# facebookresearch/pytorch3d

Measured on NVIDIA H100. Metric: rasterize frames/sec (fwd+bwd) 512^2 K=8, higher is better.
Workload: dtype f32

## Files before the change

### pytorch3d_b200/csrc/raster_meshes.cu

```cuda
#include <cfloat>
#include <climits>

#include "binning.cuh"
#include "bulk_copy.cuh"
#include "common.cuh"
#include "raster_math.cuh"

namespace b200r {

constexpr int SETUP_FACES = 256;
#ifndef B200R_MESH_TILE_H
#define B200R_MESH_TILE_H 16
#endif
constexpr int FTW = 16, FTH = B200R_MESH_TILE_H, FTHREADS = FTW * FTH;
static_assert(FTH == 16 || FTH == 8, "16x16 or 16x8 tiles");
constexpr int CHUNK = FTHREADS;
constexpr int SMEMQ_MAX_K = 32;

__device__ __forceinline__ bool face_is_drawable(const Face& f, bool cull_backfaces) {
  const float zmax = fmaxf(fmaxf(f.z0, f.z1), f.z2), zmin = fminf(fminf(f.z0, f.z1), f.z2);
  if (!(zmax >= 0.0f)) return false;
  if ((double)zmin < kEps) return false;
  const float area = edge_fn(f.x0, f.y0, f.x1, f.y1, f.x2, f.y2);
  if (cull_backfaces && area < 0.0f) return false;
// ... 916 lines not shown
      }
      store_pair_run<3 * KMAX / 4>(reinterpret_cast<float4*>(p.bary + oa * 3), piece, odd, vA, vB);
    }
    stored = true;
   }
  }
  if (!stored && valid) {
#pragma unroll
    for (int k = 0; k < KMAX; ++k) {
      if (k < K) {
        const bool e = k >= q.size;
        const float4 w = e ? make_float4(-1.f, -1.f, -1.f, -1.f) : pay[slot[k] * FTHREADS];
        p.pix_to_face[o + k] = e ? -1ll : (long long)q.id[k];
        p.zbuf[o + k] = e ? -1.0f : q.z[k];
        p.dists[o + k] = w.x;
        p.bary[(o + k) * 3 + 0] = w.y;
        p.bary[(o + k) * 3 + 1] = w.z;
        p.bary[(o + k) * 3 + 2] = w.w;
      }
    }
  }
  if (order != ORDER_ARRIVAL || !tile_saw_tie(sh)) return;
  order = ORDER_INDEX;
  rq.reset();
  }
}

__device__ __forceinline__ void recompute_hit(const FineParams& p, int fi, float px, float py, Hit& h) {
  const float4* r = p.rec + (int64_t)fi * 4;
  const float4 fa = __ldg(r + 0), fb = __ldg(r + 1), fc = __ldg(r + 2);
  const Face f = {fa.x, fa.y, fc.x, fa.z, fa.w, fc.y, fb.x, fb.y, fc.z};
  eval_pixel_face<false>(px, py, f, fb.z, p.blur_radius, p.persp != 0, p.clip != 0, false, 0.0f, h);
}

template <bool NB, bool SCAN>
__global__ void __launch_bounds__(FTHREADS, SCAN ? B200R_SMEMQ_SCAN_CTAS : B200R_SMEMQ_CTAS) mesh_fine_smemq_kernel(const FineParams p) {
  extern __shared__ __align__(16) unsigned char smem_raw[];
  FineStage& sh = *reinterpret_cast<FineStage*>(smem_raw);
  const int tid = threadIdx.x, lane = tid & 31;
  const TileWork t = tile_work(p);
  const int tile_x = t.tile_x, tile_y = t.tile_y, n = t.n;
  if (t.count == 0) {
    write_empty_tile<0>(p, n, tile_x, tile_y);
    return;
  }
  int xo, yo;
  fthread_pixel(tile_x, tile_y, xo, yo);
  const bool valid = xo < p.W && yo < p.H;
  const int lc = xo - tile_x * FTW, lr = yo - tile_y * FTH;
  const int K = p.K;

  SmemQueue<NB> q;
  q.init(smem_raw + sizeof(FineStage), K, tid);
  int order = first_walk_order<NB, SCAN>(p, t);
  bool active = valid;
  int scratch_ints = p.smem_ints;
  for (;;) {
  fine_tile_body<SmemQueue<NB>, NB, SCAN>(p, sh, q, tile_x, tile_y, n, t.seg_begin, t.count, t.overflow, order, active,
                                          scratch_ints, lc, lr);
  if (order == ORDER_DEPTH) {
    if (tile_saw_tie(sh)) {
      active = valid && sh.tie_lane[tid] != 0;
      if (active) q.reset();
      order = ORDER_INDEX;
      scratch_ints = (int)(sizeof(FineStage) / sizeof(int));
      __syncthreads();
      continue;
    }
  }
  q.sort();
  const float px = sh.col[lc], py = sh.row[lr];
  const int64_t o = (((int64_t)n * p.H + yo) * p.W + xo) * K;
  if ((K & 7) == 0) {
    const int odd = lane & 1;
    const bool vA = __shfl_sync(0xffffffffu, (int)valid, lane & ~1) != 0;
    const bool vB = __shfl_sync(0xffffffffu, (int)valid, lane | 1) != 0;
    const int64_t oa = o - (int64_t)odd * K, ob = oa + K;
    for (int g = 0; g < K; g += 8) {
      float4 pi[4], pzv[2], pd[2], pb[6];
      float z[8], d[8], b[24];
      int id[8];
#pragma unroll
      for (int u = 0; u < 8; ++u) {
        Hit h = {-1.0f, -1.0f, -1.0f, -1.0f, -1.0f};
        id[u] = -1;
        if (g + u < q.size) {
          id[u] = q.qi[(g + u) * FTHREADS];
          recompute_hit(p, id[u], px, py, h);
        }
        z[u] = h.z;
        d[u] = h.dist;
        b[3 * u + 0] = h.b0;
        b[3 * u + 1] = h.b1;
        b[3 * u + 2] = h.b2;
      }
#pragma unroll
      for (int u = 0; u < 4; ++u)
        pi[u] = make_float4(__int_as_float(id[2 * u]), __int_as_float(id[2 * u] >> 31),
                            __int_as_float(id[2 * u + 1]), __int_as_float(id[2 * u + 1] >> 31));
#pragma unroll
      for (int u = 0; u < 2; ++u) {
        pzv[u] = make_float4(z[4 * u], z[4 * u + 1], z[4 * u + 2], z[4 * u + 3]);
        pd[u] = make_float4(d[4 * u], d[4 * u + 1], d[4 * u + 2], d[4 * u + 3]);
      }
#pragma unroll
      for (int u = 0; u < 6; ++u) pb[u] = make_float4(b[4 * u], b[4 * u + 1], b[4 * u + 2], b[4 * u + 3]);
      store_pair_split<4>(reinterpret_cast<float4*>(p.pix_to_face + oa + g),
                          reinterpret_cast<float4*>(p.pix_to_face + ob + g), pi, odd, vA, vB);
      store_pair_split<2>(reinterpret_cast<float4*>(p.zbuf + oa + g), reinterpret_cast<float4*>(p.zbuf + ob + g), pzv,
                          odd, vA, vB);
      store_pair_split<2>(reinterpret_cast<float4*>(p.dists + oa + g), reinterpret_cast<float4*>(p.dists + ob + g),
                          pd, odd, vA, vB);
      store_pair_split<6>(reinterpret_cast<float4*>(p.bary + (oa + g) * 3),
                          reinterpret_cast<float4*>(p.bary + (ob + g) * 3), pb, odd, vA, vB);
    }
  } else if (valid) {
  for (int k = 0; k < K; ++k) {
    Hit h = {-1.0f, -1.0f, -1.0f, -1.0f, -1.0f};
    long long id = -1;
    if (k < q.size) {
      const int fi = q.qi[k * FTHREADS];
      recompute_hit(p, fi, px, py, h);
      id = fi;
    }
    p.pix_to_face[o + k] = id;
    p.zbuf[o + k] = h.z;
    p.dists[o + k] = h.dist;
    p.bary[(o + k) * 3 + 0] = h.b0;
    p.bary[(o + k) * 3 + 1] = h.b1;
    p.bary[(o + k) * 3 + 2] = h.b2;
  }
  }
  if (order != ORDER_ARRIVAL || !tile_saw_tie(sh)) return;
  order = ORDER_INDEX;
  q.reset();
  }
}

__global__ void __launch_bounds__(FTHREADS) mesh_fine_bigk_kernel(const FineParams p) {
  __shared__ FaceChunk s;
  const int tid = threadIdx.x, lane = tid & 31;
  const int t = blockIdx.x;
  const int n = t / (p.TY * p.TX);
  const int tile_y = (t / p.TX) % p.TY, tile_x = t % p.TX;
  int xo, yo;
  fthread_pixel(tile_x, tile_y, xo, yo);
  const bool valid = xo < p.W && yo < p.H;
  const float px = pix_to_ndc(p.W - 1 - xo, p.W, p.rx);
  const float py = pix_to_ndc(p.H - 1 - yo, p.H, p.ry);
  const float fx_lo = warp_min(valid ? px : FLT_MAX), fx_hi = warp_max(valid ? px : -FLT_MAX);
  const float fy_lo = warp_min(valid ? py : FLT_MAX), fy_hi = warp_max(valid ? py : -FLT_MAX);
  pdl_wait();
  const int seg_begin = p.tile_offset[t], seg_end = p.tile_offset[t + 1];
  const bool overflow = (int64_t)seg_end > p.capacity || seg_end == INT_MAX;
  const int64_t mesh_first = p.first[n];
  const int count = overflow ? (int)p.num[n] : seg_end - seg_begin;
  const bool persp = p.persp != 0, clip = p.clip != 0, cull = p.cull != 0;
  const int K = p.K;

  if (!overflow && count > 1)
    cta_sort_segment<FTHREADS>(p.pairs + seg_begin, count, reinterpret_cast<int*>(&s),
                               (int)(sizeof(FaceChunk) / sizeof(int)));

  float qz[B200R_MAX_K], qd[B200R_MAX_K];
  int qi[B200R_MAX_K];
  int qn = 0, q_max_idx = -1;
  float q_max_z = -1000.0f;

  for (int base = 0; base < count; base += CHUNK) {
    const int nc = min(CHUNK, count - base);
    __syncthreads();
    if (tid < nc) {
      const int f = overflow ? (int)(mesh_first + base + tid) : p.pairs[seg_begin + base + tid];
      stage_face(s, tid, p.face_verts, p.neighbor, f, p.sqrt_blur, cull);
    }
    __syncthreads();
    for (int g = 0; g < nc; g += 32) {
      bool touch = false;
      if (g + lane < nc) {
        const float4 bx = s.box[g + lane];
        touch = !(fx_lo > bx.y || fx_hi < bx.x || fy_lo > bx.w || fy_hi < bx.z);
      }
      unsigned m = __ballot_sync(0xffffffffu, touch);
      while (m) {
        const int j = g + __ffs(m) - 1;
        m &= m - 1;
        const float4 bx = s.box[j];
        if (!valid || px > bx.y || px < bx.x || py > bx.w || py < bx.z) continue;
        const float4 fa = s.a[j], fb = s.b[j], fc = s.c[j];
        const Face f = {fa.x, fa.y, fc.x, fa.z, fa.w, fc.y, fb.x, fb.y, fc.z};
        Hit h;
        const int nb = __float_as_int(fc.w);
        if (!eval_pixel_face<false>(px, py, f, fb.z, p.blur_radius, persp, clip, qn >= K && nb == -1, q_max_z, h))
          continue;
        const int fi = __float_as_int(fb.w);
        int at = -1;
        if (nb != -1)
          for (int i = 0; i < qn; ++i)
            if (qi[i] == nb) {
              at = i;
              break;
            }
        if (at >= 0) {
          if (fabsf(h.dist) < fabsf(qd[at])) {
            qz[at] = h.z;
            qi[at] = fi;
            qd[at] = h.dist;
            if (h.z > q_max_z) {
              q_max_z = h.z;
              q_max_idx = at;
            }
          }
        } else if (qn < K) {
          qz[qn] = h.z;
          qi[qn] = fi;
          qd[qn] = h.dist;
          if (h.z > q_max_z) {
            q_max_z = h.z;
            q_max_idx = qn;
          }
          ++qn;
        } else if (h.z < q_max_z) {
          qz[q_max_idx] = h.z;
          qi[q_max_idx] = fi;
          qd[q_max_idx] = h.dist;
          q_max_z = h.z;
          for (int i = 0; i < K; ++i)
            if (qz[i] > q_max_z) {
              q_max_z = qz[i];
              q_max_idx = i;
            }
        }
      }
    }
  }
  if (!valid) return;
  for (int i = 1; i < qn; ++i) {
    const float tz = qz[i];
    const int ti = qi[i];
    int j = i - 1;
    while (j >= 0 && key_less(tz, ti, qz[j], qi[j])) {
      qz[j + 1] = qz[j];
      qi[j + 1] = qi[j];
      --j;
    }
    qz[j + 1] = tz;
    qi[j + 1] = ti;
  }
  const int64_t o = (((int64_t)n * p.H + yo) * p.W + xo) * K;
  for (int k = 0; k < K; ++k) {
    Hit h = {-1.0f, -1.0f, -1.0f, -1.0f, -1.0f};
    long long id = -1;
    if (k < qn) {
      const float* v = p.face_verts + (int64_t)qi[k] * 9;
      const Face f = {__ldg(v + 0), __ldg(v + 1), __ldg(v + 2), __ldg(v + 3), __ldg(v + 4),
                      __ldg(v + 5), __ldg(v + 6), __ldg(v + 7), __ldg(v + 8)};
      eval_pixel_face<false>(px, py, f, bary_denominator(f), p.blur_radius, persp, clip, false, 0.0f, h);
      id = qi[k];
    }
    p.pix_to_face[o + k] = id;
    p.zbuf[o + k] = h.z;
    p.dists[o + k] = h.dist;
    p.bary[(o + k) * 3 + 0] = h.b0;
    p.bary[(o + k) * 3 + 1] = h.b1;
    p.bary[(o + k) * 3 + 2] = h.b2;
  }
}

struct BackwardParams {
  const float* face_verts;
  const int64_t* pix_to_face;
  const float* grad_zbuf;
  const float* grad_bary;
  const float* grad_dists;
  int N, H, W, K, TY, TX;
  int n0;
  int g_vec;
  int64_t F;
  float rx, ry;
  int persp, clip;
  float* grad_face_verts;
  const int64_t* faces;
  float* grad_verts;
  int64_t V;
};

__device__ __forceinline__ void edge_bwd(float px, float py, float ax, float ay, float bx, float by, float g,
                                         float2& dp, float2& da, float2& db) {
  dp = make_float2(g * (by - ay), g * (ax - bx));
  da = make_float2(g * (py - by), g * (bx - px));
  db = make_float2(g * (ay - py), g * (px - ax));
}

__device__ __forceinline__ void point_line_bwd(float px, float py, float ax, float ay, float bx, float by, float g,
                                               float2& ga, float2& gb) {
  const float bax = bx - ax, bay = by - ay;
  const float t = __saturatef((bax * (px - ax) + bay * (py - ay)) / (bax * bax + bay * bay));
  const float qx = (1.0f - t) * ax + t * bx, qy = (1.0f - t) * ay + t * by;
  const float cx = 2.0f * (qx - px), cy = 2.0f * (qy - py);
  ga = make_float2(g * (1.0f - t) * cx, g * (1.0f - t) * cy);
  gb = make_float2(g * t * cx, g * t * cy);
}

__device__ __forceinline__ void backward_one(const BackwardParams& p, float px, float py, int64_t fi, float gz,
                                             float gd, float gb0, float gb1, float gb2, bool persp, bool clip,
                                             float (&out)[9]) {
  const float* v = p.face_verts + fi * 9;
  const Face f = {__ldg(v + 0), __ldg(v + 1), __ldg(v + 2), __ldg(v + 3), __ldg(v + 4),
                  __ldg(v + 5), __ldg(v + 6), __ldg(v + 7), __ldg(v + 8)};
  const float den = bary_denominator(f);
  float w0, w1, w2;
  bary_coords(px, py, f, den, w0, w1, w2);
  float c0 = w0, c1 = w1, c2 = w2;
  if (persp) bary_persp(c0, c1, c2, f.z0, f.z1, f.z2);
  float k0 = c0, k1 = c1, k2 = c2;
  if (clip) bary_clip(k0, k1, k2);
  const bool inside = c0 > 0.0f && c1 > 0.0f && c2 > 0.0f;
  const float sgd = inside ? -gd : gd;

  float2 dv0 = make_float2(0.f, 0.f), dv1 = dv0, dv2 = dv0;
  {
    const float e01 = point_line_dist(px, py, f.x0, f.y0, f.x1, f.y1);
    const float e02 = point_line_dist(px, py, f.x0, f.y0, f.x2, f.y2);
    const float e12 = point_line_dist(px, py, f.x1, f.y1, f.x2, f.y2);
    if (e01 <= e02 && e01 <= e12)
      point_line_bwd(px, py, f.x0, f.y0, f.x1, f.y1, sgd, dv0, dv1);
    else if (e02 <= e01 && e02 <= e12)
      point_line_bwd(px, py, f.x0, f.y0, f.x2, f.y2, sgd, dv0, dv2);
    else if (e12 <= e01 && e12 <= e02)
      point_line_bwd(px, py, f.x1, f.y1, f.x2, f.y2, sgd, dv1, dv2);
  }

  float g0 = gb0 + gz * f.z0, g1 = gb1 + gz * f.z1, g2 = gb2 + gz * f.z2;
  if (clip) {
    const float m0 = fmaxf(c0, 0.0f), m1 = fmaxf(c1, 0.0f), m2 = fmaxf(c2, 0.0f);
    float sum = m0 + m1 + m2, gsc = 1.0f;
    if (sum < 1e-5f) {
      gsc = 0.0f;
      sum = 1e-5f;
    }
    const float inv = __frcp_rn(sum), inv2 = gsc * inv * inv;
    const float s0 = -m0 * inv2, s1 = -m1 * inv2, s2 = -m2 * inv2;
    const float cross = g0 * s0 + g1 * s1 + g2 * s2;
    const float n0 = c0 < 0.0f ? 0.0f : g0 * inv + cross;
    const float n1 = c1 < 0.0f ? 0.0f : g1 * inv + cross;
    const float n2 = c2 < 0.0f ? 0.0f : g2 * inv + cross;
    g0 = n0;
    g1 = n1;
    g2 = n2;
  }
  float dz0 = 0.0f, dz1 = 0.0f, dz2 = 0.0f;
  if (persp) {
    const float t0 = w0 * f.z1 * f.z2, t1 = f.z0 * w1 * f.z2, t2 = f.z0 * f.z1 * w2;
    const float dn = fmaxf(t0 + t1 + t2, 1e-8f);
    const float rdn = __frcp_rn(dn);
    const float gdn = (-t0 * g0 - t1 * g1 - t2 * g2) * rdn * rdn;
    const float h0 = gdn + g0 * rdn, h1 = gdn + g1 * rdn, h2 = gdn + g2 * rdn;
    g0 = h0 * f.z1 * f.z2;
    g1 = h1 * f.z0 * f.z2;
    g2 = h2 * f.z0 * f.z1;
    dz0 = h1 * w1 * f.z2 + h2 * w2 * f.z1;
    dz1 = h0 * w0 * f.z2 + h2 * w2 * f.z0;
    dz2 = h0 * w0 * f.z1 + h1 * w1 * f.z0;
  }
  float2 bv0 = make_float2(0.f, 0.f), bv1 = bv0, bv2 = bv0;
  {
    const float rden = __frcp_rn(den);
    const float e0 = edge_fn(px, py, f.x1, f.y1, f.x2, f.y2);
    const float e1 = edge_fn(px, py, f.x2, f.y2, f.x0, f.y0);
    const float e2 = edge_fn(px, py, f.x0, f.y0, f.x1, f.y1);
    float2 dp, da, db, ap, aa, ab;
    const float garea = -(g0 * e0 + g1 * e1 + g2 * e2) * rden * rden;
    edge_bwd(f.x2, f.y2, f.x0, f.y0, f.x1, f.y1, garea, ap, aa, ab);
    bv2.x += ap.x; bv2.y += ap.y;
    bv0.x += aa.x; bv0.y += aa.y;
    bv1.x += ab.x; bv1.y += ab.y;
    edge_bwd(px, py, f.x1, f.y1, f.x2, f.y2, g0 * rden, dp, da, db);
    bv1.x += da.x; bv1.y += da.y;
    bv2.x += db.x; bv2.y += db.y;
    edge_bwd(px, py, f.x2, f.y2, f.x0, f.y0, g1 * rden, dp, da, db);
    bv2.x += da.x; bv2.y += da.y;
    bv0.x += db.x; bv0.y += db.y;
    edge_bwd(px, py, f.x0, f.y0, f.x1, f.y1, g2 * rden, dp, da, db);
    bv0.x += da.x; bv0.y += da.y;
    bv1.x += db.x; bv1.y += db.y;
  }
  out[0] = bv0.x + dv0.x;
  out[1] = bv0.y + dv0.y;
  out[2] = gz * k0 + dz0;
  out[3] = bv1.x + dv1.x;
  out[4] = bv1.y + dv1.y;
  out[5] = gz * k1 + dz1;
  out[6] = bv2.x + dv2.x;
  out[7] = bv2.y + dv2.y;
  out[8] = gz * k2 + dz2;
}

__device__ __forceinline__ void red_add_v2(float* addr, float a, float b) {
  asm volatile("red.global.add.v2.f32 [%0], {%1, %2};" ::"l"(addr), "f"(a), "f"(b) : "memory");
}
__device__ __forceinline__ void warp_scatter(const BackwardParams& p, int face, float (&g)[9], int lane) {
  const unsigned grp = __match_any_sync(0xffffffffu, face);
  const unsigned above = lane == 31 ? 0u : grp & (0xffffffffu << (lane + 1));
  int next = (face >= 0 && above != 0u) ? __ffs((int)above) - 1 : -1;
  while (__any_sync(0xffffffffu, next >= 0)) {
    const int src = next >= 0 ? next : lane;
#pragma unroll
    for (int i = 0; i < 9; ++i) {
      const float v = __shfl_sync(0xffffffffu, g[i], src);
      if (next >= 0) g[i] += v;
    }
    const int nn = __shfl_sync(0xffffffffu, next, src);
    next = next >= 0 ? nn : -1;
  }
  if (face >= 0 && lane == __ffs((int)grp) - 1) {
    if (p.faces != nullptr) {
      const int64_t* fc = p.faces + (int64_t)face * 3;
#pragma unroll
      for (int j = 0; j < 3; ++j) {
        const int64_t vi = __ldg(fc + j);
        if (vi < 0 || vi >= p.V) continue;
        float* o = p.grad_verts + vi * 3;
#ifndef B200R_EXP_BWD_SCALAR_RED
        if (p.g_vec) {
          const bool odd = (vi & 1) != 0;
          const float s1 = odd ? g[3 * j] : g[3 * j + 2];
          const float a = odd ? g[3 * j + 1] : g[3 * j], b = odd ? g[3 * j + 2] : g[3 * j + 1];
          if (s1 != 0.0f) atomicAdd(o + (odd ? 0 : 2), s1);
          if (a != 0.0f || b != 0.0f) red_add_v2(o + (odd ? 1 : 0), a, b);
          continue;
        }
#endif
#pragma unroll
        for (int c = 0; c < 3; ++c)
          if (g[3 * j + c] != 0.0f) atomicAdd(o + c, g[3 * j + c]);
      }
    } else {
      float* o = p.grad_face_verts + (int64_t)face * 9;
#ifndef B200R_EXP_BWD_SCALAR_RED
      if (p.g_vec) {
        const int odd = face & 1;
        atomicAdd(o + (odd ? 0 : 8), odd ? g[0] : g[8]);
#pragma unroll
        for (int j = 0; j < 4; ++j)
          red_add_v2(o + 2 * j + odd, odd ? g[2 * j + 1] : g[2 * j], odd ? g[2 * j + 2] : g[2 * j + 1]);
        return;
      }
#endif
#pragma unroll
      for (int i = 0; i < 9; ++i) atomicAdd(o + i, g[i]);
    }
  }
}

#ifndef B200R_BWD_PF_CTAS
#define B200R_BWD_PF_CTAS 3
#endif
#ifndef B200R_BWD_CTAS
#define B200R_BWD_CTAS 4
#endif
template <int GV, bool PF>
__global__ void __launch_bounds__(TILE_THREADS, PF ? B200R_BWD_PF_CTAS : B200R_BWD_CTAS) mesh_backward_kernel(const BackwardParams p) {
  const int lane = threadIdx.x & 31;
  const int tile_x = blockIdx.x, tile_y = blockIdx.y, n = p.n0 + blockIdx.z;
  int xo, yo;
  thread_pixel(tile_x, tile_y, xo, yo);
  const bool in_image = xo < p.W && yo < p.H;
  const float px = pix_to_ndc(p.W - 1 - xo, p.W, p.rx);
  const float py = pix_to_ndc(p.H - 1 - yo, p.H, p.ry);
  const int K = p.K;
  const int64_t o = in_image ? (((int64_t)n * p.H + yo) * p.W + xo) * K : 0;
  const bool persp = p.persp != 0, clip = p.clip != 0;
  constexpr int G = GV > 0 ? GV : 1;
  static_assert(!PF || GV == 8, "the prefetching variant is the K % 8 == 0 kernel");

  for (int k0 = 0; k0 < K; k0 += G) {
    int fk[G];
    if (GV > 0) {
#pragma unroll
      for (int k = 0; k < G; k += 2) {
        longlong2 v = make_longlong2(-1, -1);
        if (in_image) v = __ldg(reinterpret_cast<const longlong2*>(p.pix_to_face + o + k0 + k));
        fk[k] = (int)v.x;
        fk[k + 1] = (int)v.y;
      }
    } else {
      fk[0] = in_image ? (int)p.pix_to_face[o + k0] : -1;
    }
    float pz[PF ? 4 : 1], pd[PF ? 4 : 1], pb[PF ? 12 : 1];
    if (PF) {
      float4 vz = make_float4(0.f, 0.f, 0.f, 0.f), vd = vz, b0 = vz, b1 = vz, b2 = vz;
      if (fk[0] >= 0) {
        vz = __ldg(reinterpret_cast<const float4*>(p.grad_zbuf + o + k0));
        vd = __ldg(reinterpret_cast<const float4*>(p.grad_dists + o + k0));
        const float4* gb = reinterpret_cast<const float4*>(p.grad_bary + (o + k0) * 3);
        b0 = __ldg(gb + 0);
        b1 = __ldg(gb + 1);
        b2 = __ldg(gb + 2);
      }
      pz[0] = vz.x; pz[1] = vz.y; pz[2] = vz.z; pz[3] = vz.w;
      pd[0] = vd.x; pd[1] = vd.y; pd[2] = vd.z; pd[3] = vd.w;
      pb[0] = b0.x; pb[1] = b0.y; pb[2] = b0.z; pb[3] = b0.w;
      pb[4] = b1.x; pb[5] = b1.y; pb[6] = b1.z; pb[7] = b1.w;
      pb[8] = b2.x; pb[9] = b2.y; pb[10] = b2.z; pb[11] = b2.w;
    }
#pragma unroll 1
    for (int j = 0; j < G; ++j) {
      const int face = fk[0];
#pragma unroll
      for (int u = 0; u + 1 < G; ++u) fk[u] = fk[u + 1];
      float gz = 0.f, gd = 0.f, gb0 = 0.f, gb1 = 0.f, gb2 = 0.f;
      if (PF) {
        gz = pz[0]; gd = pd[0]; gb0 = pb[0]; gb1 = pb[1]; gb2 = pb[2];
#pragma unroll
        for (int u = 0; u < 3; ++u) {
          pz[u] = pz[u + 1];
          pd[u] = pd[u + 1];
        }
#pragma unroll
        for (int u = 0; u < 9; ++u) pb[u] = pb[u + 3];
      }
      if (!__any_sync(0xffffffffu, face >= 0)) continue;
      float g[9] = {0.f, 0.f, 0.f, 0.f, 0.f, 0.f, 0.f, 0.f, 0.f};
      if (face >= 0) {
        const int64_t i = o + k0 + j;
        if (!PF || j >= 4) {
          gz = __ldg(p.grad_zbuf + i);
          gd = __ldg(p.grad_dists + i);
          gb0 = __ldg(p.grad_bary + i * 3);
          gb1 = __ldg(p.grad_bary + i * 3 + 1);
          gb2 = __ldg(p.grad_bary + i * 3 + 2);
        }
        backward_one(p, px, py, face, gz, gd, gb0, gb1, gb2, persp, clip, g);
      }
      warp_scatter(p, face, g, lane);
    }
  }
}

}

__global__ void __launch_bounds__(256) mesh_gather_kernel(const float* __restrict__ verts, int64_t V,
                                                          const int64_t* __restrict__ faces, int64_t F,
                                                          float* __restrict__ face_verts_out) {
  const int64_t e = (int64_t)blockIdx.x * blockDim.x + threadIdx.x;
  if (e >= F * 3) return;
  const int64_t vi = __ldg(faces + e);
  const bool ok = vi >= 0 && vi < V;
#pragma unroll
  for (int c = 0; c < 3; ++c) face_verts_out[e * 3 + c] = ok ? __ldg(verts + vi * 3 + c) : __int_as_float(0x7fc00000);
}

using namespace b200r;

extern "C" size_t b200r_rasterize_meshes_workspace_bytes(int64_t F, int32_t N, int32_t H, int32_t W,
                                                         int64_t pair_capacity) {
  if (F < 0 || N < 0 || H < 0 || W < 0) return 0;
  return carve_workspace(nullptr, F, N, H, W, pair_capacity, FTH, FTW).bytes +
         FACE_RECORD_BYTES * (size_t)(F > 0 ? F : 1);
}

static int forward_impl(const float* face_verts, const float* verts, int64_t V, const int64_t* faces,
                        float* face_verts_out, int64_t F, const int64_t* first, const int64_t* num,
                        const int64_t* neighbor, int32_t N, int32_t H, int32_t W, float blur_radius, int32_t K,
                        int32_t perspective_correct, int32_t clip_barycentric_coords, int32_t cull_backfaces,
                        int64_t* pix_to_face, float* zbuf, float* bary, float* dists, void* workspace,
                        size_t workspace_bytes, int64_t pair_capacity, void* stream_) {
  cudaStream_t stream = static_cast<cudaStream_t>(stream_);
  if (K > B200R_MAX_K) return fail(B200R_ERR_INVALID_ARGUMENT, "Must have points_per_pixel <= 150");
  if (F < 0 || N < 0 || H < 0 || W < 0 || K < 0) return fail(B200R_ERR_INVALID_ARGUMENT, "negative size");
  if (F > INT_MAX) return fail(B200R_ERR_INVALID_ARGUMENT, "more than 2^31-1 packed faces are not supported");
  if ((int64_t)N * H * W * K == 0) return B200R_OK;
  const int TY = div_up(H, FTH), TX = div_up(W, FTW);
  if (TY > 0xFFFE || TX > 0xFFFE) return fail(B200R_ERR_INVALID_ARGUMENT, "image too large");
  const int64_t ntiles = (int64_t)N * TY * TX;
  if (ntiles > INT_MAX) return fail(B200R_ERR_INVALID_ARGUMENT, "too many tiles");
  BinWorkspace ws = carve_workspace(workspace, F, N, H, W, pair_capacity, FTH, FTW);
  const size_t nrec = (size_t)(F > 0 ? F : 1);
  if (workspace == nullptr || workspace_bytes < ws.bytes + FACE_RECORD_BYTES * nrec)
    return fail(B200R_ERR_WORKSPACE, "workspace too small for rasterize_meshes_forward");
  float4* rec = reinterpret_cast<float4*>(static_cast<char*>(workspace) + ws.bytes);

  const float rx = ndc_range(W, H), ry = ndc_range(H, W);
  const float sqrt_blur = sqrtf(blur_radius);

  const bool prof = profiling_enabled();
  if (prof) phase_timer().record(0, stream);
#ifndef B200R_EXP_MEMSET_NODE
  zero_ints_kernel<<<(unsigned)((ntiles + 1023) / 1024), 256, 0, stream>>>(ws.tile_count, ntiles);
  B200R_LAUNCHED("zero_ints_kernel");
#else
  B200R_CUDA_OK(cudaMemsetAsync(ws.tile_count, 0, sizeof(int) * (size_t)ntiles, stream));
#endif
  if (F > 0) {
    const unsigned sgrid = (unsigned)((F + SETUP_FACES - 1) / SETUP_FACES);
#ifndef B200R_EXP_MEMSET_NODE
#define B200R_SETUP_LAUNCH(KERNEL, ...) B200R_CUDA_OK(launch_chained(KERNEL, dim3(sgrid), dim3(SETUP_FACES), 0, stream, __VA_ARGS__))
#else
#define B200R_SETUP_LAUNCH(KERNEL, ...) KERNEL<<<sgrid, SETUP_FACES, 0, stream>>>(__VA_ARGS__)
#endif
    if (faces != nullptr) {
      B200R_SETUP_LAUNCH(mesh_setup_count_kernel<true>, (const float*)nullptr, verts, V, faces, face_verts_out, neighbor, F,
                         first, num, N, H, W, TY, TX, rx, ry, sqrt_blur, cull_backfaces, ws.rect, ws.tile_count, rec);
      face_verts = face_verts_out;
    } else {
      B200R_SETUP_LAUNCH(mesh_setup_count_kernel<false>, face_verts, (const float*)nullptr, (int64_t)0,
                         (const int64_t*)nullptr, (float*)nullptr, neighbor, F, first, num, N, H, W, TY, TX, rx, ry,
                         sqrt_blur, cull_backfaces, ws.rect, ws.tile_count, rec);
    }
#undef B200R_SETUP_LAUNCH
    B200R_LAUNCHED("mesh_setup_count_kernel");
  }
#ifdef B200R_EXP_NOTILEORDER
  int* const tile_order = nullptr;
#else
  int* const tile_order = (blur_radius > 0.0f && ntiles < (1ll << ORDER_BITS)) ? ws.tile_order : nullptr;
#endif
  B200R_CUDA_OK(launch_chained(tile_scan_kernel, dim3(1), dim3(1024), 0, stream, ws.tile_count, ws.tile_offset,
                               (int)ntiles, tile_order));
  B200R_LAUNCHED("tile_scan_kernel");
  if (F > 0) {
    B200R_CUDA_OK(launch_chained(tile_fill_kernel<true>, dim3((unsigned)((F + 255) / 256)), dim3(256), 0, stream,
                                 ws.rect, F, TY, TX, ws.tile_count, ws.pairs, ws.capacity));
    B200R_LAUNCHED("tile_fill_kernel");
  }
  if (prof) phase_timer().record(1, stream);
  FineParams p;
  p.face_verts = face_verts;
  p.neighbor = neighbor;
  p.rec = rec;
  p.n0 = 0;
  p.first = first;
  p.num = num;
  p.tile_offset = ws.tile_offset;
  p.tile_order = tile_order;
  p.pairs = ws.pairs;
  p.capacity = ws.capacity;
  p.N = N; p.H = H; p.W = W; p.K = K; p.TY = TY; p.TX = TX;
  p.rx = rx; p.ry = ry; p.blur_radius = blur_radius; p.sqrt_blur = sqrt_blur;
  p.persp = perspective_correct; p.clip = clip_barycentric_coords; p.cull = cull_backfaces;
  p.smem_ints = 0;
  p.pix_to_face = pix_to_face; p.zbuf = zbuf; p.bary = bary; p.dists = dists;
  const unsigned grid = (unsigned)ntiles;
  const bool no_blur = !(blur_radius > 0.0f);
  int dev_ = 0;
  B200R_CUDA_OK(cudaGetDevice(&dev_));
#define B200R_FINE_LAUNCH(KERNEL, SMEM_MAX, SMEM)                                                         \
  do {                                                                                                   \
    static bool configured[64] = {};                                                                     \
    if (dev_ < 0 || dev_ >= 64 || !configured[dev_]) {                                                   \
      B200R_CUDA_OK(cudaFuncSetAttribute(KERNEL, cudaFuncAttributeMaxDynamicSharedMemorySize, (int)(SMEM_MAX))); \
      if (dev_ >= 0 && dev_ < 64) configured[dev_] = true;                                               \
    }                                                                                                    \
    p.smem_ints = (int)((SMEM) / sizeof(int));                                                           \
    for (p.n0 = 0; p.n0 < N; p.n0 += 65535) {                                                            \
      const dim3 grid3((unsigned)TX, (unsigned)TY, (unsigned)min(N - p.n0, 65535));                      \
      B200R_CUDA_OK(launch_chained(KERNEL, grid3, dim3(FTHREADS), (SMEM), stream, p));                   \
    }                                                                                                    \
  } while (0)
#define B200R_FINE(KM)                                                                                    \
  do {                                                                                                   \
    constexpr size_t smem_ = sizeof(FineStage) + sizeof(float4) * KM * FTHREADS;                         \
    if (neighbor && no_blur)                                                                             \
      B200R_FINE_LAUNCH((mesh_fine_kernel<KM, true, true>), smem_, smem_);                               \
    else if (neighbor)                                                                                   \
      B200R_FINE_LAUNCH((mesh_fine_kernel<KM, true, false>), smem_, smem_);                              \
    else if (no_blur)                                                                                    \
      B200R_FINE_LAUNCH((mesh_fine_kernel<KM, false, true>), smem_, smem_);                              \
    else                                                                                                 \
      B200R_FINE_LAUNCH((mesh_fine_kernel<KM, false, false>), smem_, smem_);                             \
  } while (0)
  if (K <= 1)
    B200R_FINE(1);
  else if (K <= 2)
    B200R_FINE(2);
  else if (K <= 4)
    B200R_FINE(4);
  else if (K <= 8)
    B200R_FINE(8);
  else if (K <= SMEMQ_MAX_K) {
    const size_t smem_max_nb = sizeof(FineStage) + (size_t)SMEMQ_MAX_K * FTHREADS * 12;
    const size_t smem_max = sizeof(FineStage) + (size_t)SMEMQ_MAX_K * FTHREADS * 8;
    const size_t smem_nb = sizeof(FineStage) + (size_t)K * FTHREADS * 12;
    const size_t smem = sizeof(FineStage) + (size_t)K * FTHREADS * 8;
    if (neighbor && no_blur)
      B200R_FINE_LAUNCH((mesh_fine_smemq_kernel<true, true>), smem_max_nb, smem_nb);
    else if (neighbor)
      B200R_FINE_LAUNCH((mesh_fine_smemq_kernel<true, false>), smem_max_nb, smem_nb);
    else if (no_blur)
      B200R_FINE_LAUNCH((mesh_fine_smemq_kernel<false, true>), smem_max, smem);
    else
      B200R_FINE_LAUNCH((mesh_fine_smemq_kernel<false, false>), smem_max, smem);
  } else
    B200R_CUDA_OK(launch_chained(mesh_fine_bigk_kernel, dim3(grid), dim3(FTHREADS), 0, stream, p));
#undef B200R_FINE
#undef B200R_FINE_LAUNCH
  B200R_LAUNCHED("mesh_fine_kernel");
  if (prof) {
    phase_timer().record(2, stream);
    phase_timer().have_fwd = true;
  }
  return B200R_OK;
}

extern "C" int b200r_rasterize_meshes_forward(const float* face_verts, int64_t F, const int64_t* first,
                                              const int64_t* num, const int64_t* neighbor, int32_t N, int32_t H,
                                              int32_t W, float blur_radius, int32_t K, int32_t bin_size,
                                              int32_t max_faces_per_bin, int32_t perspective_correct,
                                              int32_t clip_barycentric_coords, int32_t cull_backfaces,
                                              int64_t* pix_to_face, float* zbuf, float* bary, float* dists,
                                              void* workspace, size_t workspace_bytes, int64_t pair_capacity,
                                              void* stream_) {
  (void)bin_size;
  (void)max_faces_per_bin;
  return forward_impl(face_verts, nullptr, 0, nullptr, nullptr, F, first, num, neighbor, N, H, W, blur_radius, K,
                      perspective_correct, clip_barycentric_coords, cull_backfaces, pix_to_face, zbuf, bary, dists,
                      workspace, workspace_bytes, pair_capacity, stream_);
}

extern "C" int b200r_rasterize_meshes_forward_indexed(const float* verts, int64_t V, const int64_t* faces, int64_t F,
                                                      const int64_t* first, const int64_t* num,
                                                      const int64_t* neighbor, int32_t N, int32_t H, int32_t W,
                                                      float blur_radius, int32_t K, int32_t perspective_correct,
                                                      int32_t clip_barycentric_coords, int32_t cull_backfaces,
                                                      int64_t* pix_to_face, float* zbuf, float* bary, float* dists,
                                                      float* face_verts_out, void* workspace,
                                                      size_t workspace_bytes, int64_t pair_capacity,
                                                      void* stream_) {
  if (V < 0) return fail(B200R_ERR_INVALID_ARGUMENT, "negative size");
  if (F > 0 && (faces == nullptr || face_verts_out == nullptr || (V > 0 && verts == nullptr)))
    return fail(B200R_ERR_INVALID_ARGUMENT, "verts, faces and face_verts_out must not be null");
  if ((int64_t)N * H * W * K == 0 && F > 0) {
    cudaStream_t stream = static_cast<cudaStream_t>(stream_);
    mesh_gather_kernel<<<(unsigned)((F * 3 + 255) / 256), 256, 0, stream>>>(verts, V, faces, F, face_verts_out);
    B200R_LAUNCHED("mesh_gather_kernel");
    return B200R_OK;
  }
  return forward_impl(nullptr, verts, V, F > 0 ? faces : nullptr, face_verts_out, F, first, num, neighbor, N, H, W,
                      blur_radius, K, perspective_correct, clip_barycentric_coords, cull_backfaces, pix_to_face,
                      zbuf, bary, dists, workspace, workspace_bytes, pair_capacity, stream_);
}

static int backward_impl(const float* face_verts, int64_t F, const int64_t* pix_to_face, const float* grad_zbuf,
                         const float* grad_bary, const float* grad_dists, int32_t N, int32_t H, int32_t W, int32_t K,
                         int32_t perspective_correct, int32_t clip_barycentric_coords, float* grad_face_verts,
                         const int64_t* faces, float* grad_verts, int64_t V, void* stream_) {
  cudaStream_t stream = static_cast<cudaStream_t>(stream_);
  if (F < 0 || N < 0 || H < 0 || W < 0 || K < 0) return fail(B200R_ERR_INVALID_ARGUMENT, "negative size");
  if (F == 0) return B200R_OK;
  if (faces == nullptr) B200R_CUDA_OK(cudaMemsetAsync(grad_face_verts, 0, sizeof(float) * 9 * (size_t)F, stream));
  if ((int64_t)N * H * W * K == 0) return B200R_OK;
  const int TY = div_up(H, TILE), TX = div_up(W, TILE);
  BackwardParams p;
  p.face_verts = face_verts; p.pix_to_face = pix_to_face;
  p.grad_zbuf = grad_zbuf; p.grad_bary = grad_bary; p.grad_dists = grad_dists;
  p.N = N; p.H = H; p.W = W; p.K = K; p.TY = TY; p.TX = TX;
  p.F = F;
  p.g_vec = (reinterpret_cast<uintptr_t>(faces != nullptr ? grad_verts : grad_face_verts) & 7u) == 0 ? 1 : 0;
  p.rx = ndc_range(W, H); p.ry = ndc_range(H, W);
  p.persp = perspective_correct; p.clip = clip_barycentric_coords;
  p.grad_face_verts = grad_face_verts;
  p.faces = faces;
  p.grad_verts = grad_verts;
  p.V = V;
  const bool prof = profiling_enabled();
  if (prof) phase_timer().record(3, stream);
  for (p.n0 = 0; p.n0 < N; p.n0 += 65535) {
    const dim3 bgrid((unsigned)TX, (unsigned)TY, (unsigned)min(N - p.n0, 65535));
    const bool aligned = ((reinterpret_cast<uintptr_t>(grad_zbuf) | reinterpret_cast<uintptr_t>(grad_bary) |
                           reinterpret_cast<uintptr_t>(grad_dists)) & 15u) == 0;
#ifdef B200R_EXP_BWDPF
    const bool prefetch = aligned;
#else
    const bool prefetch = false && aligned;
#endif
    if ((K & 7) == 0 && prefetch)
      mesh_backward_kernel<8, true><<<bgrid, TILE_THREADS, 0, stream>>>(p);
    else if ((K & 7) == 0)
      mesh_backward_kernel<8, false><<<bgrid, TILE_THREADS, 0, stream>>>(p);
    else if ((K & 3) == 0)
      mesh_backward_kernel<4, false><<<bgrid, TILE_THREADS, 0, stream>>>(p);
    else
      mesh_backward_kernel<0, false><<<bgrid, TILE_THREADS, 0, stream>>>(p);
  }
  B200R_LAUNCHED("mesh_backward_kernel");
  if (prof) {
    phase_timer().record(4, stream);
    phase_timer().have_bwd = true;
  }
  return B200R_OK;
}

extern "C" int b200r_rasterize_meshes_backward(const float* face_verts, int64_t F, const int64_t* pix_to_face,
                                               const float* grad_zbuf, const float* grad_bary,
                                               const float* grad_dists, int32_t N, int32_t H, int32_t W, int32_t K,
                                               int32_t perspective_correct, int32_t clip_barycentric_coords,
                                               float* grad_face_verts, void* stream_) {
  return backward_impl(face_verts, F, pix_to_face, grad_zbuf, grad_bary, grad_dists, N, H, W, K, perspective_correct,
                       clip_barycentric_coords, grad_face_verts, nullptr, nullptr, 0, stream_);
}

extern "C" int b200r_rasterize_meshes_backward_indexed(const float* face_verts, const int64_t* faces, int64_t F,
                                                       int64_t V, const int64_t* pix_to_face,
                                                       const float* grad_zbuf, const float* grad_bary,
                                                       const float* grad_dists, int32_t N, int32_t H, int32_t W,
                                                       int32_t K, int32_t perspective_correct,
                                                       int32_t clip_barycentric_coords, float* grad_verts,
                                                       float* grad_face_verts_scratch, void* stream_) {
  cudaStream_t stream = static_cast<cudaStream_t>(stream_);
  if (F < 0 || V < 0) return fail(B200R_ERR_INVALID_ARGUMENT, "negative size");
  if (V > 0) B200R_CUDA_OK(cudaMemsetAsync(grad_verts, 0, sizeof(float) * 3 * (size_t)V, stream));
  if (F == 0 || V == 0) return B200R_OK;
  (void)grad_face_verts_scratch;
  return backward_impl(face_verts, F, pix_to_face, grad_zbuf, grad_bary, grad_dists, N, H, W, K, perspective_correct,
                       clip_barycentric_coords, nullptr, faces, grad_verts, V, stream_);
}
```

Measured before the change: 18580.

## Overlap gradient zeroing with backward kernel via programmatic dependent launch

Replaces the cudaMemsetAsync of the gradient buffer with a custom zeroing kernel that triggers programmatic dependent launch. The backward kernel is launched chained and only waits on the zeroing before its first atomic scatter, so face loads and barycentric math can overlap the memset. It also drops the unused prefetch variant, lowers the CTA-per-SM bound to 3 and adds alignment checks for vectorized index loads. The risk is extra launch setup per call and lower occupancy from the changed launch bound.

```diff
diff --git a/pytorch3d_b200/csrc/raster_meshes.cu b/pytorch3d_b200/csrc/raster_meshes.cu
--- a/pytorch3d_b200/csrc/raster_meshes.cu
+++ b/pytorch3d_b200/csrc/raster_meshes.cu
@@ -1242,12 +1242,8 @@
   gb = make_float2(g * t * cx, g * t * cy);
 }
 
-__device__ __forceinline__ void backward_one(const BackwardParams& p, float px, float py, int64_t fi, float gz,
-                                             float gd, float gb0, float gb1, float gb2, bool persp, bool clip,
-                                             float (&out)[9]) {
-  const float* v = p.face_verts + fi * 9;
-  const Face f = {__ldg(v + 0), __ldg(v + 1), __ldg(v + 2), __ldg(v + 3), __ldg(v + 4),
-                  __ldg(v + 5), __ldg(v + 6), __ldg(v + 7), __ldg(v + 8)};
+__device__ __forceinline__ void backward_one(float px, float py, const Face& f, float gz, float gd, float gb0,
+                                             float gb1, float gb2, bool persp, bool clip, float (&out)[9]) {
   const float den = bary_denominator(f);
   float w0, w1, w2;
   bary_coords(px, py, f, den, w0, w1, w2);
@@ -1393,14 +1389,11 @@
   }
 }
 
-#ifndef B200R_BWD_PF_CTAS
-#define B200R_BWD_PF_CTAS 3
-#endif
 #ifndef B200R_BWD_CTAS
-#define B200R_BWD_CTAS 4
-#endif
-template <int GV, bool PF>
-__global__ void __launch_bounds__(TILE_THREADS, PF ? B200R_BWD_PF_CTAS : B200R_BWD_CTAS) mesh_backward_kernel(const BackwardParams p) {
+#define B200R_BWD_CTAS 3
+#endif
+template <int GV>
+__global__ void __launch_bounds__(TILE_THREADS, B200R_BWD_CTAS) mesh_backward_kernel(const BackwardParams p) {
   const int lane = threadIdx.x & 31;
   const int tile_x = blockIdx.x, tile_y = blockIdx.y, n = p.n0 + blockIdx.z;
   int xo, yo;
@@ -1412,7 +1405,7 @@
   const int64_t o = in_image ? (((int64_t)n * p.H + yo) * p.W + xo) * K : 0;
   const bool persp = p.persp != 0, clip = p.clip != 0;
   constexpr int G = GV > 0 ? GV : 1;
-  static_assert(!PF || GV == 8, "the prefetching variant is the K % 8 == 0 kernel");
+  bool waited = false;
 
   for (int k0 = 0; k0 < K; k0 += G) {
     int fk[G];
@@ -1427,55 +1420,60 @@
     } else {
       fk[0] = in_image ? (int)p.pix_to_face[o + k0] : -1;
     }
-    float pz[PF ? 4 : 1], pd[PF ? 4 : 1], pb[PF ? 12 : 1];
-    if (PF) {
-      float4 vz = make_float4(0.f, 0.f, 0.f, 0.f), vd = vz, b0 = vz, b1 = vz, b2 = vz;
-      if (fk[0] >= 0) {
-        vz = __ldg(reinterpret_cast<const float4*>(p.grad_zbuf + o + k0));
-        vd = __ldg(reinterpret_cast<const float4*>(p.grad_dists + o + k0));
-        const float4* gb = reinterpret_cast<const float4*>(p.grad_bary + (o + k0) * 3);
-        b0 = __ldg(gb + 0);
-        b1 = __ldg(gb + 1);
-        b2 = __ldg(gb + 2);
-      }
-      pz[0] = vz.x; pz[1] = vz.y; pz[2] = vz.z; pz[3] = vz.w;
-      pd[0] = vd.x; pd[1] = vd.y; pd[2] = vd.z; pd[3] = vd.w;
-      pb[0] = b0.x; pb[1] = b0.y; pb[2] = b0.z; pb[3] = b0.w;
-      pb[4] = b1.x; pb[5] = b1.y; pb[6] = b1.z; pb[7] = b1.w;
-      pb[8] = b2.x; pb[9] = b2.y; pb[10] = b2.z; pb[11] = b2.w;
-    }
+#ifdef B200R_EXP_BWD_IDX_ONLY
+    {
+      int acc = 0;
+#pragma unroll
+      for (int k = 0; k < G; ++k) acc ^= fk[k];
+      if (acc == 0x7ffffffe) p.grad_face_verts[0] = 1.0f;
+      continue;
+    }
+#endif
 #pragma unroll 1
     for (int j = 0; j < G; ++j) {
       const int face = fk[0];
 #pragma unroll
       for (int u = 0; u + 1 < G; ++u) fk[u] = fk[u + 1];
-      float gz = 0.f, gd = 0.f, gb0 = 0.f, gb1 = 0.f, gb2 = 0.f;
-      if (PF) {
-        gz = pz[0]; gd = pd[0]; gb0 = pb[0]; gb1 = pb[1]; gb2 = pb[2];
-#pragma unroll
-        for (int u = 0; u < 3; ++u) {
-          pz[u] = pz[u + 1];
-          pd[u] = pd[u + 1];
-        }
-#pragma unroll
-        for (int u = 0; u < 9; ++u) pb[u] = pb[u + 3];
-      }
       if (!__any_sync(0xffffffffu, face >= 0)) continue;
       float g[9] = {0.f, 0.f, 0.f, 0.f, 0.f, 0.f, 0.f, 0.f, 0.f};
       if (face >= 0) {
         const int64_t i = o + k0 + j;
-        if (!PF || j >= 4) {
-          gz = __ldg(p.grad_zbuf + i);
-          gd = __ldg(p.grad_dists + i);
-          gb0 = __ldg(p.grad_bary + i * 3);
-          gb1 = __ldg(p.grad_bary + i * 3 + 1);
-          gb2 = __ldg(p.grad_bary + i * 3 + 2);
-        }
-        backward_one(p, px, py, face, gz, gd, gb0, gb1, gb2, persp, clip, g);
+        const float gz = __ldg(p.grad_zbuf + i);
+        const float gd = __ldg(p.grad_dists + i);
+        const float gb0 = __ldg(p.grad_bary + i * 3);
+        const float gb1 = __ldg(p.grad_bary + i * 3 + 1);
+        const float gb2 = __ldg(p.grad_bary + i * 3 + 2);
+        const float* v = p.face_verts + (int64_t)face * 9;
+        const Face f = {__ldg(v + 0), __ldg(v + 1), __ldg(v + 2), __ldg(v + 3), __ldg(v + 4),
+                        __ldg(v + 5), __ldg(v + 6), __ldg(v + 7), __ldg(v + 8)};
+        backward_one(px, py, f, gz, gd, gb0, gb1, gb2, persp, clip, g);
+      }
+#ifdef B200R_EXP_BWD_NOSCATTER
+      if (g[0] + g[1] + g[2] + g[3] + g[4] + g[5] + g[6] + g[7] + g[8] == 1234.5f) p.grad_face_verts[0] = 1.0f;
+      continue;
+#endif
+      if (!waited) {
+        pdl_wait();
+        waited = true;
       }
       warp_scatter(p, face, g, lane);
     }
   }
+  if (!waited) pdl_wait();
+}
+
+#ifndef B200R_ZERO_CTAS
+#define B200R_ZERO_CTAS 1
+#endif
+__global__ void __launch_bounds__(256) zero_floats_kernel(float* __restrict__ p, int64_t n) {
+  pdl_trigger();
+  const int64_t i = (int64_t)blockIdx.x * 256 + threadIdx.x, stride = (int64_t)gridDim.x * 256;
+  const int64_t head = min((int64_t)(((16u - (reinterpret_cast<uintptr_t>(p) & 15u)) & 15u) >> 2), n);
+  const int64_t nv = (n - head) >> 2, tail = head + nv * 4;
+  float4* q = reinterpret_cast<float4*>(p + head);
+  for (int64_t j = i; j < nv; j += stride) q[j] = make_float4(0.f, 0.f, 0.f, 0.f);
+  if (i < head) p[i] = 0.0f;
+  if (i < n - tail) p[tail + i] = 0.0f;
 }
 
 }
@@ -1681,47 +1679,52 @@
                       zbuf, bary, dists, workspace, workspace_bytes, pair_capacity, stream_);
 }
 
+static int zero_floats(float* p, int64_t n, cudaStream_t stream) {
+  if (n <= 0) return B200R_OK;
+  int dev = 0, sms = 0;
+  B200R_CUDA_OK(cudaGetDevice(&dev));
+  B200R_CUDA_OK(cudaDeviceGetAttribute(&sms, cudaDevAttrMultiProcessorCount, dev));
+  const int64_t blocks = std::min<int64_t>((n / 4 + 255) / 256 + 1, B200R_ZERO_CTAS * (int64_t)std::max(sms, 1));
+  zero_floats_kernel<<<(unsigned)blocks, 256, 0, stream>>>(p, n);
+  B200R_LAUNCHED("zero_floats_kernel");
+  return B200R_OK;
+}
+
 static int backward_impl(const float* face_verts, int64_t F, const int64_t* pix_to_face, const float* grad_zbuf,
                          const float* grad_bary, const float* grad_dists, int32_t N, int32_t H, int32_t W, int32_t K,
                          int32_t perspective_correct, int32_t clip_barycentric_coords, float* grad_face_verts,
                          const int64_t* faces, float* grad_verts, int64_t V, void* stream_) {
   cudaStream_t stream = static_cast<cudaStream_t>(stream_);
-  if (F < 0 || N < 0 || H < 0 || W < 0 || K < 0) return fail(B200R_ERR_INVALID_ARGUMENT, "negative size");
-  if (F == 0) return B200R_OK;
-  if (faces == nullptr) B200R_CUDA_OK(cudaMemsetAsync(grad_face_verts, 0, sizeof(float) * 9 * (size_t)F, stream));
-  if ((int64_t)N * H * W * K == 0) return B200R_OK;
+  if (F < 0 || N < 0 || H < 0 || W < 0 || K < 0 || V < 0) return fail(B200R_ERR_INVALID_ARGUMENT, "negative size");
+  float* const target = faces != nullptr ? grad_verts : grad_face_verts;
+  const int64_t target_n = faces != nullptr ? 3 * V : 9 * F;
+  const bool draw = F > 0 && target_n > 0 && (int64_t)N * H * W * K > 0;
+  const bool prof = draw && profiling_enabled();
+  if (prof) phase_timer().record(3, stream);
+  if (const int rc = zero_floats(target, target_n, stream)) return rc;
+  if (!draw) return B200R_OK;
   const int TY = div_up(H, TILE), TX = div_up(W, TILE);
   BackwardParams p;
   p.face_verts = face_verts; p.pix_to_face = pix_to_face;
   p.grad_zbuf = grad_zbuf; p.grad_bary = grad_bary; p.grad_dists = grad_dists;
   p.N = N; p.H = H; p.W = W; p.K = K; p.TY = TY; p.TX = TX;
   p.F = F;
-  p.g_vec = (reinterpret_cast<uintptr_t>(faces != nullptr ? grad_verts : grad_face_verts) & 7u) == 0 ? 1 : 0;
+  p.g_vec = (reinterpret_cast<uintptr_t>(target) & 7u) == 0 ? 1 : 0;
   p.rx = ndc_range(W, H); p.ry = ndc_range(H, W);
   p.persp = perspective_correct; p.clip = clip_barycentric_coords;
   p.grad_face_verts = grad_face_verts;
   p.faces = faces;
   p.grad_verts = grad_verts;
   p.V = V;
-  const bool prof = profiling_enabled();
-  if (prof) phase_timer().record(3, stream);
+  const bool idx_vec = (reinterpret_cast<uintptr_t>(pix_to_face) & 15u) == 0;
   for (p.n0 = 0; p.n0 < N; p.n0 += 65535) {
     const dim3 bgrid((unsigned)TX, (unsigned)TY, (unsigned)min(N - p.n0, 65535));
-    const bool aligned = ((reinterpret_cast<uintptr_t>(grad_zbuf) | reinterpret_cast<uintptr_t>(grad_bary) |
-                           reinterpret_cast<uintptr_t>(grad_dists)) & 15u) == 0;
-#ifdef B200R_EXP_BWDPF
-    const bool prefetch = aligned;
-#else
-    const bool prefetch = false && aligned;
-#endif
-    if ((K & 7) == 0 && prefetch)
-      mesh_backward_kernel<8, true><<<bgrid, TILE_THREADS, 0, stream>>>(p);
-    else if ((K & 7) == 0)
-      mesh_backward_kernel<8, false><<<bgrid, TILE_THREADS, 0, stream>>>(p);
-    else if ((K & 3) == 0)
-      mesh_backward_kernel<4, false><<<bgrid, TILE_THREADS, 0, stream>>>(p);
+    if ((K & 7) == 0 && idx_vec)
+      B200R_CUDA_OK(launch_chained(mesh_backward_kernel<8>, bgrid, dim3(TILE_THREADS), 0, stream, p));
+    else if ((K & 3) == 0 && idx_vec)
+      B200R_CUDA_OK(launch_chained(mesh_backward_kernel<4>, bgrid, dim3(TILE_THREADS), 0, stream, p));
     else
-      mesh_backward_kernel<0, false><<<bgrid, TILE_THREADS, 0, stream>>>(p);
+      B200R_CUDA_OK(launch_chained(mesh_backward_kernel<0>, bgrid, dim3(TILE_THREADS), 0, stream, p));
   }
   B200R_LAUNCHED("mesh_backward_kernel");
   if (prof) {
@@ -1747,10 +1750,8 @@
                                                        int32_t K, int32_t perspective_correct,
                                                        int32_t clip_barycentric_coords, float* grad_verts,
                                                        float* grad_face_verts_scratch, void* stream_) {
-  cudaStream_t stream = static_cast<cudaStream_t>(stream_);
   if (F < 0 || V < 0) return fail(B200R_ERR_INVALID_ARGUMENT, "negative size");
-  if (V > 0) B200R_CUDA_OK(cudaMemsetAsync(grad_verts, 0, sizeof(float) * 3 * (size_t)V, stream));
-  if (F == 0 || V == 0) return B200R_OK;
+  if (F == 0 || V == 0) return zero_floats(grad_verts, 3 * V, static_cast<cudaStream_t>(stream_));
   (void)grad_face_verts_scratch;
   return backward_impl(face_verts, F, pix_to_face, grad_zbuf, grad_bary, grad_dists, N, H, W, K, perspective_correct,
                        clip_barycentric_coords, nullptr, faces, grad_verts, V, stream_);
```

Result: faster. 18770, median of 6 (+1.0%).
